# OedonLestrange42/GNURadio-WiFI-ImageTransfer

Hardware: AMD Instinct MI355X
Metric: OFDM demod throughput (complex samples/s), 802.11a RX chain sync->LLR (higher is better)
Workload: dtype f32

## Files before the change

gnuradio-wifi-imagetransfer_amd/csrc/wifirx_api.hip:

```cpp
#include <hip/hip_runtime.h>
#include <emmintrin.h>

#include <algorithm>
#include <array>
#include <atomic>
#include <chrono>
#include <cmath>
#include <cstdio>
#include <cstdlib>
#include <cstring>
#include <condition_variable>
#include <deque>
#include <memory>
#include <mutex>
#include <new>
#include <optional>
#include <thread>
#include <string>
#include <vector>

#include "wifirx.h"
#include "wr_kernels.h"
#include "wr_tx.h"
#include "wr_channel.h"
// ... 38 lines not shown
        p = nullptr;
        bytes = 0;
    }
    int alloc(wifirx_handle* h, size_t n, const char* what)
    {
        reset();
        hipError_t e = Pinned ? hipHostMalloc(&p, n, hipHostMallocDefault) : hipMalloc(&p, n);
        if (e != hipSuccess) { p = nullptr; return oom(h, what, e); }
        bytes = n;
        return WIFIRX_OK;
    }
    int reserve(wifirx_handle* h, size_t need)
    {
        if (bytes >= need) return WIFIRX_OK;
        return Pinned ? alloc(h, need + need / 2, "hipHostMalloc") : alloc(h, need, "hipMalloc");
    }
};
using DevBuf = Buffer<false>;
using PinnedBuf = Buffer<true>;

struct Tunables {
    int32_t  llr_csi = 0;
    int32_t  llr_format = WIFIRX_LLR_F32;
    int32_t  stream_want_idx = 1;
    int32_t  stream_soft = 0;
    int64_t  stream_batch = 0;
    uint32_t decode_small_max = WR_DECODE_SMALL_MAX;
};

struct Environment {
    uint32_t decode_fpw = 0;
    int      decode_ovl = -1;
    int      decode_q = -1;
    int      fail_alloc = 0, alloc_count = 0;
    size_t   decode_budget = 0;
    int      fail_decode_scratch = 0;
    int      fail_carry = 0, carry_count = 0;
};

struct Staging {
    DevBuf iq, frames, idx, llr, car, csi, stats, hbits;
    DevBuf off;
    DevBuf tx_psdu, tx_meta;
    DevBuf ch_meta;
    DevBuf link_meta, link_payload;
    DevBuf link_counts;
    DevBuf iq_clipped;
};

struct DecodeWork {
    DevBuf scratch, max;
    DevBuf perm;
    DevBuf hbits;
};

struct StreamState {
    DevBuf   sbuf;
    DevBuf   native;
    DevBuf   above, A;
    int64_t  sbuf_cap = 0;
    int64_t  sbase = 0;
    int64_t  sfill = 0;
    int64_t  sdetected = 0;
    int64_t  sprocessed = 0;
    int64_t  last_trig = -(1ll << 40);
    std::vector<PendingTrig> pending;
    std::deque<PolledFrame>  queue;
    std::atomic<uint32_t> n_queued{0};
    DevBuf   trig, frames, idx, car, psdu, csi, stats, hbits;
    uint32_t out_cap = 0;
    DevBuf   llr;
    DevBuf   pack;
    PinnedBuf host;
    bool     dead = false;
    std::string dead_msg;
    size_t   push_consumed = 0;
};

struct Job { const void* ptr; size_t n; bool flush; int fmt; float scale; };

struct Worker {
    mutable std::mutex      mu;
    std::condition_variable cv;
    std::thread             thread;
    bool    stop = false, busy = false;
    std::optional<Job> job;
// ... 23 lines not shown
};

namespace {

thread_local std::string g_err;
thread_local bool t_is_worker = false;

int fail(wifirx_handle* h, int code, const std::string& msg)
{
    if (h) { if (t_is_worker) h->w.err_local = msg; else h->err = msg; }
    g_err = msg;
    return code;
}

#define HIP_TRY(h, expr)                                                                       \
    do {                                                                                       \
        hipError_t e_ = (expr);                                                                \
        if (e_ != hipSuccess)                                                                  \
            return fail(h, WIFIRX_EHIP, std::string(#expr) + ": " + hipGetErrorString(e_));   \
    } while (0)

int oom(wifirx_handle* h, const char* what, hipError_t e)
{
    (void)hipGetLastError();
    return fail(h, WIFIRX_ENOMEM, std::string(what) + ": " + hipGetErrorString(e));
}

int read_environment(wifirx_handle* h)
{
    Environment& v = h->env;
    if (const char* e = std::getenv("WIFIRX_DECODE_SMALL_MAX")) h->tune.decode_small_max = (uint32_t)std::strtoul(e, nullptr, 10);
    if (const char* e = std::getenv("WIFIRX_DECODE_FPW")) v.decode_fpw = (uint32_t)std::strtoul(e, nullptr, 10);
    if (const char* e = std::getenv("WIFIRX_DECODE_Q")) v.decode_q = std::atoi(e) != 0;
    if (const char* e = std::getenv("WIFIRX_DECODE_OVL")) { const int m = std::atoi(e); if (m == 0 || m == 2) v.decode_ovl = m; }
    if (const char* e = std::getenv("WIFIRX_TEST_FAIL_ALLOC")) v.fail_alloc = std::atoi(e);
    if (const char* e = std::getenv("WIFIRX_TEST_FAIL_CARRY")) v.fail_carry = std::atoi(e);
    if (const char* e = std::getenv("WIFIRX_TEST_DECODE_BUDGET")) v.decode_budget = (size_t)std::strtoull(e, nullptr, 10);
    if (const char* e = std::getenv("WIFIRX_TEST_FAIL_DECODE_SCRATCH")) v.fail_decode_scratch = std::atoi(e);
    int prio = 0, prio_lo = 0, prio_hi = 0;
    if (const char* e = std::getenv("WIFIRX_STREAM_PRIORITY")) {
        if (hipDeviceGetStreamPriorityRange(&prio_lo, &prio_hi) == hipSuccess) prio = e[0] == 'h' ? prio_hi : e[0] == 'l' ? prio_lo : 0;
        else (void)hipGetLastError();
    }
    return prio;
}

wr::DemodParams params_of(const wifirx_handle* h)
{
    wr::DemodParams p;
    p.bandwidth = h->cfg.bandwidth;
    p.frequency = h->cfg.frequency;
    p.threshold = h->cfg.sensitivity;
    p.min_plateau = h->cfg.min_plateau;
    p.max_sym = h->cfg.max_sym;
    p.llr_bits = h->cfg.llr_bits;
    p.chan_est = h->cfg.chan_est;
    p.llr_csi = h->tune.llr_csi;
    return p;
}

}

static void stream_worker_stop(wifirx_handle* h);
static void stream_worker_wait_idle(wifirx_handle* h);

extern "C" {
// ... 334 lines not shown
```

gnuradio-wifi-imagetransfer_amd/csrc/wifirx_api_decode.inc:

```
static int decode_batch_impl(wifirx_handle* h, uint32_t n_slots, const wifirx_out* out);

extern "C" int wifirx_decode_batch(wifirx_handle* h, uint32_t n_slots, const wifirx_out* out)
{
    if (!h || !out) return WIFIRX_EINVAL;
    stream_worker_wait_idle(h);
    return decode_batch_impl(h, n_slots, out);
}


static int decode_prepass(wifirx_handle* h, uint32_t n_slots, const wifirx_out* out, uint32_t (&pre)[9])
{
    HIP_TRY(h, hipSetDevice(h->device));
    int rc = h->dec.max.reserve(h, 256);
    if (rc) return rc;
    HIP_TRY(h, hipMemsetAsync(h->dec.max.p, 0, 256, h->stream));
    HIP_TRY(h, wr_launch_decode_maxsteps(h->stream, n_slots, h->cfg.max_sym, out->frames, out->psdu_stride,
                                         h->dec.max.as<uint32_t>()));
    HIP_TRY(h, hipMemcpyAsync(pre, h->dec.max.p, sizeof pre, hipMemcpyDeviceToHost, h->stream));
    HIP_TRY(h, hipStreamSynchronize(h->stream));
    return WIFIRX_OK;
}

struct DecodeGroups { uint32_t starts[9]; uint32_t n_virtual; const uint32_t* perm; };

static int decode_group_by_rate(wifirx_handle* h, uint32_t n_slots, const wifirx_out* out, const uint32_t (&pre)[9],
                                uint32_t fpw, DecodeGroups& g)
{
    uint32_t n_rates = 0;
    g.starts[0] = 0;
    for (int e = 0; e < 8; e++) {
        n_rates += pre[1 + e] != 0;
        g.starts[e + 1] = g.starts[e] + (pre[1 + e] + fpw - 1) / fpw * fpw;
    }
    g.n_virtual = n_rates > 1 ? g.starts[8] : n_slots;
    g.perm = nullptr;
    if (n_rates <= 1) return WIFIRX_OK;
    int rc = h->dec.perm.reserve(h, (size_t)g.n_virtual * sizeof(uint32_t));
    if (rc) return rc;
    HIP_TRY(h, hipMemsetAsync(h->dec.perm.p, 0xff, (size_t)g.n_virtual * sizeof(uint32_t), h->stream));
    HIP_TRY(h, wr_launch_decode_perm(h->stream, n_slots, h->cfg.max_sym, out->frames, out->psdu_stride, g.starts,
                                     h->dec.max.as<uint32_t>() + 16, h->dec.perm.as<uint32_t>()));
    g.perm = h->dec.perm.as<const uint32_t>();
    return WIFIRX_OK;
}

static size_t decode_scratch_budget(wifirx_handle* h)
{
    size_t budget = WR_DECODE_SCRATCH_BUDGET;
    size_t mem_free = 0, mem_total = 0;
    if (hipMemGetInfo(&mem_free, &mem_total) == hipSuccess) budget = std::min<size_t>(budget, (mem_free + h->dec.scratch.bytes) / 10 * 7);
    else (void)hipGetLastError();
    if (h->env.decode_budget) budget = std::min<size_t>(budget, h->env.decode_budget);
    return budget;
}

static int decode_alloc_scratch(wifirx_handle* h, size_t stride, size_t want, size_t budget, size_t& n_waves)
{
    n_waves = std::max<size_t>(1, std::min<size_t>(want, budget / stride));
    for (;;) {
        int rc;
        if (h->env.fail_decode_scratch > 0 && h->env.fail_decode_scratch-- > 0) {
            DevBuf none;
            rc = none.reserve(h, SIZE_MAX / 2);
            if (rc == WIFIRX_OK) rc = fail(h, WIFIRX_ENOMEM, "hipMalloc(decode scratch): test hook");
        } else {
            rc = h->dec.scratch.reserve(h, stride * n_waves);
        }
        if (rc == WIFIRX_OK) return WIFIRX_OK;
        if (rc != WIFIRX_ENOMEM || n_waves <= 4) return rc;
        n_waves /= 2;
    }
}

static int decode_batch_impl(wifirx_handle* h, uint32_t n_slots, const wifirx_out* out)
{
    if (!h || !out) return WIFIRX_EINVAL;
    if (!out->on_device) return fail(h, WIFIRX_EINVAL, "wifirx_decode_batch works on device buffers (out->on_device = 1)");
    if (!out->frames || (!out->idx && !out->hbits) || !out->psdu || out->psdu_stride == 0)
        return fail(h, WIFIRX_EINVAL, "frames, hbits or idx, and psdu (with psdu_stride) are required");
    if (reinterpret_cast<uintptr_t>(out->hbits) & 15) return fail(h, WIFIRX_EINVAL, "out->hbits must be 16-byte aligned");
    if (n_slots == 0) return WIFIRX_OK;
    uint32_t pre[9] = { 0 };
    int rc = decode_prepass(h, n_slots, out, pre);
    if (rc || pre[0] == 0) return rc;
    const uint32_t n_steps = pre[0];
    const uint32_t* hbits = out->hbits;
    if (!hbits) {
        rc = h->dec.hbits.reserve(h, (size_t)n_slots * h->cfg.max_sym * 48);
        if (rc) return rc;
        HIP_TRY(h, wr_launch_decode_pack(h->stream, n_slots, h->cfg.max_sym, out->frames, out->idx, out->psdu_stride,
                                         h->dec.hbits.as<uint32_t>(), n_steps));
        hbits = h->dec.hbits.as<const uint32_t>();
    }
    if (n_slots <= h->tune.decode_small_max) {
        const size_t stride = wr::dec_small_slice(n_steps);
        const size_t n_waves = std::min<size_t>(n_slots, WR_DECODE_MAX_WAVES);
        rc = h->dec.scratch.reserve(h, stride * n_waves);
        if (rc) return rc;
        HIP_TRY(h, wr_launch_decode_small(h->stream, n_slots, h->cfg.max_sym, out->frames, hbits, out->psdu,
                                          out->psdu_stride, h->dec.scratch.as<uint8_t>(), stride, n_steps,
                                          (uint32_t)n_waves));
        return WIFIRX_OK;
    }
    uint32_t n_dec = 0;
    for (int e = 0; e < 8; e++) n_dec += pre[1 + e];
    const bool use_q = h->env.decode_q == 1 || (h->env.decode_q < 0 && n_dec >= WR_DECODE_Q_MIN_FRAMES);
    const uint32_t fpw_max = use_q ? WR_DECODE_Q_FRAMES_PER_WAVE : WR_DECODE_FRAMES_PER_WAVE;
    size_t stride = use_q ? wr::dec_q_slice(n_steps, false) : wr::dec_pair_slice(n_steps);
    uint32_t fpw = (uint32_t)std::min<size_t>(fpw_max, std::max<size_t>(1, (n_slots + 1023) / 1024));
    if (use_q && h->env.decode_q < 0) fpw = fpw_max;
    if (h->env.decode_fpw) fpw = std::min<uint32_t>(fpw_max, h->env.decode_fpw);
    DecodeGroups g;
    if ((rc = decode_group_by_rate(h, n_slots, out, pre, fpw, g))) return rc;
    const size_t n_tasks = (g.n_virtual + fpw - 1) / fpw;
    size_t budget = decode_scratch_budget(h);
    const size_t stride_spec = wr::dec_q_slice(n_steps, true);
    const size_t spec_waves = (size_t)h->n_simd * ((pre[7] | pre[8]) ? 2 : WR_DQ_SPEC_WAVES);
    int mode = 0;
    if (use_q) {
        if (h->env.decode_ovl >= 0) mode = h->env.decode_ovl;
        else if (n_tasks >= WR_DECODE_MAX_WAVES / 2 && budget / stride_spec >= spec_waves) mode = 2;
    }
    if (mode == 2) stride = stride_spec;
    size_t n_waves = 0;
    if ((rc = decode_alloc_scratch(h, stride, std::min<size_t>(n_tasks, mode == 2 ? spec_waves : WR_DECODE_MAX_WAVES), budget, n_waves)))
        return rc;
    if (use_q)
        HIP_TRY(h, wr_launch_decode_q(h->stream, n_slots, h->cfg.max_sym, out->frames, hbits, out->psdu,
                                      out->psdu_stride, h->dec.scratch.as<uint8_t>(), stride, n_steps,
                                      (uint32_t)n_waves, fpw, g.perm, g.n_virtual, (pre[7] | pre[8]) != 0, mode));
    else
        HIP_TRY(h, wr_launch_decode(h->stream, n_slots, h->cfg.max_sym, out->frames, hbits, out->psdu,
                                    out->psdu_stride, h->dec.scratch.as<uint8_t>(), stride, n_steps,
                                    (uint32_t)n_waves, fpw, g.perm, g.n_virtual));
    return WIFIRX_OK;
}

static int decode_batch_soft_impl(wifirx_handle* h, uint32_t n_slots, const wifirx_out* out, uint32_t llr_bits, bool bf16);

extern "C" int wifirx_decode_batch_soft(wifirx_handle* h, uint32_t n_slots, const wifirx_out* out)
{
    if (!h || !out) return WIFIRX_EINVAL;
    stream_worker_wait_idle(h);
    if (h->cfg.llr_bits == 0) return fail(h, WIFIRX_EINVAL, "wifirx_decode_batch_soft needs a handle created with llr_bits > 0");
    return decode_batch_soft_impl(h, n_slots, out, h->cfg.llr_bits, h->tune.llr_format == WIFIRX_LLR_BF16);
}

static int decode_batch_soft_impl(wifirx_handle* h, uint32_t n_slots, const wifirx_out* out, uint32_t llr_bits, bool bf16)
{
    if (!out->on_device) return fail(h, WIFIRX_EINVAL, "wifirx_decode_batch_soft works on device buffers (out->on_device = 1)");
    if (!out->frames || !out->llr || !out->psdu || out->psdu_stride == 0)
        return fail(h, WIFIRX_EINVAL, "frames, llr and psdu (with psdu_stride) are required");
    if (reinterpret_cast<uintptr_t>(out->llr) & 15) return fail(h, WIFIRX_EINVAL, "out->llr must be 16-byte aligned");
    if (n_slots == 0) return WIFIRX_OK;
    uint32_t pre[9] = { 0 };
    int rc = decode_prepass(h, n_slots, out, pre);
    if (rc || pre[0] == 0) return rc;
    const uint32_t n_steps = pre[0];
    const uint32_t fpw = 64;
// ... 26 lines not shown
```

gnuradio-wifi-imagetransfer_amd/csrc/wr_decode.h:

```cpp
#pragma once
#include <hip/hip_runtime.h>
#include <stdint.h>

#include "wifirx.h"

namespace wr {

constexpr int RATE_NDBPS[8] = { 24, 36, 48, 72, 96, 144, 192, 216 };
constexpr __host__ __device__ int ndbps_of(int enc) { return RATE_NDBPS[enc]; }
constexpr __host__ __device__ int nbpsc_of(int enc) { return enc < 2 ? 1 : enc < 4 ? 2 : enc < 6 ? 4 : 6; }
constexpr __host__ __device__ int punct_of(int enc) { return enc == 6 ? 1 : (enc & 1) ? 2 : 0; }
constexpr __host__ __device__ int words_per_sym(int enc) { return 2 * nbpsc_of(enc); }

__device__ __forceinline__ int frame_steps(uint32_t flags, int enc, int len, uint32_t psdu_stride, uint32_t max_sym,
                                           uint32_t n_steps_cap)
{
    const int n_dbps = ndbps_of(enc & 7);
    const int n_sym = (16 + 8 * len + 6 + n_dbps - 1) / n_dbps;
    const bool ok = (flags & WIFIRX_F_COMPLETE) && len <= (int)psdu_stride && len <= WIFIRX_MAX_PSDU &&
                    n_sym <= WIFIRX_MAX_SYM && n_sym <= (int)max_sym && (uint32_t)(n_sym * n_dbps) <= n_steps_cap;
    return ok ? n_sym * n_dbps : 0;
}

constexpr int coded_index(int punct, int n_bpsc, int ci)
{
    const int n_cbps = 48 * n_bpsc;
    const int s = (n_bpsc / 2) < 1 ? 1 : (n_bpsc / 2);
    int k = ci;
    if (punct == 1) {
        const int r = ci & 3;
        if (r == 3) return -1;
        k = (ci >> 2) * 3 + r;
    } else if (punct == 2) {
        const int g = ci / 6, r = ci - 6 * g;
        if (r == 3 || r == 4) return -1;
        k = g * 4 + (r < 3 ? r : 3);
    }
    const int i = (n_cbps >> 4) * (k & 15) + (k >> 4);
    return s * (i / s) + (i + n_cbps - (16 * i) / n_cbps) % s;
}

constexpr __host__ __device__ int rotr6(int s, int p) { return ((s >> p) | (s << (6 - p))) & 63; }
constexpr __host__ __device__ int parity_of(int v) { return __builtin_popcount(v) & 1; }

constexpr int RATE_TAB_STRIDE = 216;
struct RateTable { uint32_t e[8 * RATE_TAB_STRIDE]; };
template <typename Entry>
constexpr RateTable make_rate_table(Entry entry)
{
    RateTable t{};
    for (int enc = 0; enc < 8; enc++)
        for (int tt = 0; tt < RATE_TAB_STRIDE; tt++) {
            const int nb = nbpsc_of(enc), pu = punct_of(enc);
            const bool in = tt < ndbps_of(enc);
            const int ja = in ? coded_index(pu, nb, 2 * tt) : -1, jb = in ? coded_index(pu, nb, 2 * tt + 1) : -1;
            t.e[enc * RATE_TAB_STRIDE + tt] = entry(nb, ja) | (entry(nb, jb) << 16);
        }
    return t;
}

struct FinishTables { uint32_t crc[4][256]; uint32_t scr[128]; };

__device__ __forceinline__ void build_finish_tables(FinishTables& ft)
{
    for (int e = threadIdx.x; e < 256; e += blockDim.x) {
        uint32_t c = (uint32_t)e;
#pragma unroll
        for (int k = 0; k < 8; k++) c = (c >> 1) ^ (0xedb88320u & (0u - (c & 1u)));
        ft.crc[0][e] = c;
    }
    __syncthreads();
    for (int e = threadIdx.x; e < 256; e += blockDim.x) {
// ... 61 lines not shown
```

gnuradio-wifi-imagetransfer_amd/csrc/wr_decode.hip:

```cpp
#include <hip/hip_runtime.h>
#include <stdint.h>
#include <type_traits>

#include "wifirx.h"
#include "wr_kernels.h"
#include "wr_decode.h"

namespace wr {

#define WR_DEC_WAVES_PER_SIMD 4
#define WR_DEC_CHUNK      60
#define WR_DEC_NORM_STEPS 120

#define WR_SRC_PUNCT 0x200u
constexpr int bin_of_carrier(int c)
{
    int i = c + 6;
    if (i >= 11) i++;
    if (i >= 25) i++;
    if (i >= 32) i++;
    if (i >= 39) i++;
    if (i >= 53) i++;
    return i;
}
constexpr uint32_t coded_src(int n_bpsc, int j)
{
    if (j < 0) return WR_SRC_PUNCT;
    const int carrier = j / n_bpsc, bit = j - carrier * n_bpsc;
    const int bin = bin_of_carrier(carrier);
    return (uint32_t)(bin & 31) | ((uint32_t)(2 * bit + (bin >> 5)) << 5);
}
__constant__ const RateTable WR_SRC_TABLE = make_rate_table(coded_src);

__device__ __forceinline__ void copy_src_table(uint32_t* tab)
{
    for (int e = threadIdx.x; e < 8 * RATE_TAB_STRIDE; e += blockDim.x) tab[e] = WR_SRC_TABLE.e[e];
}

__device__ __forceinline__ void gather_step(const uint32_t* tile, int sym0, int n_words, const uint32_t* __restrict__ tab_enc,
                                            int n_dbps, uint32_t recip, int t, bool in_range, int& ra, int& rb)
{
    ra = 2; rb = 2;
    if (in_range) {
        const int sym = (int)__umulhi((uint32_t)t, recip);
        const int tt = t - sym * n_dbps;
        const uint32_t e = tab_enc[tt];
        const uint32_t ea = e & 0xffffu, eb = e >> 16;
        const uint32_t* sp = tile + (sym - sym0) * n_words;
        if (!(ea & WR_SRC_PUNCT)) ra = (int)((sp[(ea >> 5) & 15u] >> (ea & 31u)) & 1u);
        if (!(eb & WR_SRC_PUNCT)) rb = (int)((sp[(eb >> 5) & 15u] >> (eb & 31u)) & 1u);
    }
}

#define WR_RECIP32(d) (uint32_t)((0x100000000ull + (d) - 1) / (d))

template <int NB>
__device__ __forceinline__ void pack_symbol(const uint32_t (&by)[12], uint32_t* __restrict__ dst)
{
    uint32_t w[2 * NB];
#pragma unroll
    for (int k = 0; k < 2 * NB; k++) w[k] = 0;
#pragma unroll
    for (int c = 0; c < 48; c++) {
        const int bin = bin_of_carrier(c);
// ... 737 lines not shown
                if (SPEC && blk > 0) {
                    const uint32_t S = rec[(size_t)blk * 64 + lane];
                    bool joined = true;
#pragma unroll
                    for (int h = 0; h < 4; h++) joined = joined && st[h] == (int)((S >> (8 * h)) & 63u) && fb[h] >= blk;
                    if (__all(joined)) break;
                }
            }
#undef WR_DQ_PICK
        }
        __threadfence_block();
#pragma unroll
        for (int h = 0; h < 4; h++) {
            if (n_data[h] > 0) {
                const uint32_t slot = slot_of[h];
                finish_frame<256>(dbits + 64 * h + lane, frames[slot].psdu_len, psdu_all + (size_t)slot * psdu_stride,
                                  ((reinterpret_cast<uintptr_t>(psdu_all) | psdu_stride) & 3) == 0, frames + slot, frames[slot].flags, ft);
            }
        }
    }
}

__device__ __forceinline__ uint32_t crc32_update(uint32_t c, uint32_t byte)
{
    c ^= byte;
#pragma unroll
    for (int k = 0; k < 8; k++) c = (c >> 1) ^ (0xedb88320u & (0u - (c & 1u)));
    return c;
}

__global__ __launch_bounds__(256)
void decode_small_kernel(uint32_t n_slots, uint32_t max_sym, wifirx_frame* __restrict__ frames,
                         const uint32_t* __restrict__ hbits_all, uint8_t* __restrict__ psdu_all, uint32_t psdu_stride,
                         uint8_t* __restrict__ scratch, size_t scratch_stride, uint32_t n_steps_cap, uint32_t n_waves_total)
{
    __shared__ uint32_t tile_all[4][60 * 12];
    __shared__ uint32_t src_tab[8 * RATE_TAB_STRIDE];
    copy_src_table(src_tab);
    __syncthreads();
    const int lane = threadIdx.x & 63;
    const int wv = threadIdx.x >> 6;
    const uint32_t wave = blockIdx.x * 4 + wv;
    if (wave >= n_waves_total) return;
    uint32_t* tile = tile_all[wv];
    uint8_t* const slice = scratch + (size_t)wave * scratch_stride;
    uint64_t* dec = reinterpret_cast<uint64_t*>(slice);
    uint64_t* words = reinterpret_cast<uint64_t*>(slice + dec_small_words_at(n_steps_cap));

    const int s = lane, u = s & 1, p0 = s >> 1, p1 = (s >> 1) | 32;
    const int f0 = (p0 << 1) | u;
    const int a0 = __builtin_popcount(f0 & 0155) & 1, b0 = __builtin_popcount(f0 & 0117) & 1;
    const uint32_t recip_tab[8] = { WR_RECIP32(24), WR_RECIP32(36), WR_RECIP32(48), WR_RECIP32(72),
                                    WR_RECIP32(96), WR_RECIP32(144), WR_RECIP32(192), WR_RECIP32(216) };

    for (uint32_t slot = wave; slot < n_slots; slot += n_waves_total) {
        const wifirx_frame fr = frames[slot];
        const int enc = fr.encoding & 7, psdu_len = fr.psdu_len;
        const int n_data = frame_steps(fr.flags, enc, psdu_len, psdu_stride, max_sym, n_steps_cap);
        if (n_data == 0) continue;
        const int n_dbps = ndbps_of(enc);
        const int n_sym = __builtin_amdgcn_readfirstlane(n_data / n_dbps);
        const int n_words = words_per_sym(enc);
        const uint32_t* fhb = hbits_all + (size_t)slot * max_sym * 12;
        const uint32_t recip = recip_tab[enc];
        const uint32_t* tab_enc = src_tab + enc * RATE_TAB_STRIDE;

        int pm = (s == 0) ? 0 : (1 << 24);
        for (int sym0 = 0; sym0 < n_sym; sym0 += 60) {
            const int nsy = n_sym - sym0 < 60 ? n_sym - sym0 : 60;
            const int nw = nsy * n_words;
            __builtin_amdgcn_wave_barrier();
            for (int o = lane; o < nw; o += 64) tile[o] = fhb[sym0 * n_words + o];
            __builtin_amdgcn_wave_barrier();
            const int t_hi = (sym0 + nsy) * n_dbps;
            for (int t0 = sym0 * n_dbps; t0 < t_hi; t0 += WR_DEC_CHUNK) {
                const int t = t0 + lane;
                int ra, rb;
                gather_step(tile, sym0, n_words, tab_enc, n_dbps, recip, t, lane < WR_DEC_CHUNK && t < t_hi, ra, rb);
                const uint64_t A1 = __ballot(ra == 1), AV = __ballot(ra != 2);
                const uint64_t B1 = __ballot(rb == 1), BV = __ballot(rb != 2);
                const int jn = t_hi - t0 < WR_DEC_CHUNK ? t_hi - t0 : WR_DEC_CHUNK;
                uint64_t mydec = 0;
                for (int j = 0; j < jn; j++) {
                    const int sa = (int)((A1 >> j) & 1), va = (int)((AV >> j) & 1);
                    const int sb = (int)((B1 >> j) & 1), vb = (int)((BV >> j) & 1);
                    const int bm0 = (va & (sa ^ a0)) + (vb & (sb ^ b0));
                    const int bm1 = (va + vb) - bm0;
                    const int m0 = __shfl(pm, p0, 64) + bm0;
                    const int m1 = __shfl(pm, p1, 64) + bm1;
                    const bool sel = m1 < m0;
                    pm = sel ? m1 : m0;
                    const uint64_t d = __ballot(sel);
// ... 71 lines not shown
                            uint32_t psdu_stride, uint32_t* __restrict__ out)
{
    uint32_t best = 0;
    uint32_t cnt[8] = { 0, 0, 0, 0, 0, 0, 0, 0 };
    const uint32_t n_round = (n_slots + 63u) & ~63u;
    for (uint32_t i = blockIdx.x * blockDim.x + threadIdx.x; i < n_round; i += gridDim.x * blockDim.x) {
        int enc = -1;
        if (i < n_slots) {
            const wifirx_frame fr = frames[i];
            const uint32_t v = (uint32_t)frame_steps(fr.flags, fr.encoding & 7, fr.psdu_len, psdu_stride, max_sym, 0xffffffffu);
            if (v) {
                best = v > best ? v : best;
                enc = fr.encoding & 7;
            }
        }
#pragma unroll
        for (int e = 0; e < 8; e++) cnt[e] += (uint32_t)__builtin_popcountll(__ballot(enc == e));
    }
#pragma unroll
    for (int k = 1; k < 64; k <<= 1) {
        uint32_t o = __shfl_xor(best, k, 64);
        best = o > best ? o : best;
    }
    if ((threadIdx.x & 63) == 0) {
        if (best) atomicMax(out, best);
#pragma unroll
        for (int e = 0; e < 8; e++) if (cnt[e]) atomicAdd(out + 1 + e, cnt[e]);
    }
}

struct PermStarts { uint32_t s[8]; };
__global__ __launch_bounds__(256)
void decode_perm_kernel(uint32_t n_slots, uint32_t max_sym, const wifirx_frame* __restrict__ frames, uint32_t psdu_stride,
                        PermStarts start, uint32_t* __restrict__ cursor, uint32_t* __restrict__ perm)
{
    const int lane = threadIdx.x & 63;
    const uint32_t n_round = (n_slots + 63u) & ~63u;
    for (uint32_t i = blockIdx.x * blockDim.x + threadIdx.x; i < n_round; i += gridDim.x * blockDim.x) {
        int enc = -1;
        if (i < n_slots) {
            const wifirx_frame fr = frames[i];
            if (frame_steps(fr.flags, fr.encoding & 7, fr.psdu_len, psdu_stride, max_sym, 0xffffffffu)) enc = fr.encoding & 7;
        }
#pragma unroll
        for (int e = 0; e < 8; e++) {
            const uint64_t m = __ballot(enc == e);
            if (m == 0) continue;
            uint32_t at = 0;
            if (lane == (int)__builtin_ctzll(m)) at = atomicAdd(cursor + e, (uint32_t)__builtin_popcountll(m));
            at = (uint32_t)__builtin_amdgcn_readlane((int)at, (int)__builtin_ctzll(m));
            if (enc == e) perm[start.s[e] + at + (uint32_t)__builtin_popcountll(m & ((1ull << lane) - 1ull))] = i;
        }
    }
}

}

extern "C" hipError_t wr_launch_decode_maxsteps(hipStream_t st, uint32_t n_slots, uint32_t max_sym,
                                                const wifirx_frame* frames, uint32_t psdu_stride, uint32_t* out)
{
    if (n_slots == 0) return hipSuccess;
    uint32_t blocks = (n_slots + 255) / 256;
    if (blocks > 1024) blocks = 1024;
    hipLaunchKernelGGL(wr::decode_maxsteps_kernel, dim3(blocks), dim3(256), 0, st, n_slots, max_sym, frames, psdu_stride, out);
    return hipGetLastError();
}

extern "C" hipError_t wr_launch_decode_pack(hipStream_t st, uint32_t n_slots, uint32_t max_sym, const wifirx_frame* frames,
                                            const uint8_t* idx, uint32_t psdu_stride, uint32_t* hbits, uint32_t n_steps_cap)
{
    if (n_slots == 0) return hipSuccess;
    uint32_t blocks = (n_slots + 3) / 4;
    if (blocks > 16384) blocks = 16384;
    hipLaunchKernelGGL(wr::decode_pack_kernel, dim3(blocks), dim3(256), 0, st, n_slots, max_sym, frames, idx, psdu_stride,
                       hbits, n_steps_cap);
    return hipGetLastError();
}

extern "C" hipError_t wr_launch_decode(hipStream_t st, uint32_t n_slots, uint32_t max_sym, wifirx_frame* frames,
                                       const uint32_t* hbits, uint8_t* psdu, uint32_t psdu_stride, uint8_t* scratch,
                                       size_t scratch_stride, uint32_t n_steps_cap, uint32_t n_waves, uint32_t frames_per_wave,
                                       const uint32_t* perm, uint32_t n_virtual)
{
    if (n_slots == 0 || n_waves == 0) return hipSuccess;
    if (!perm) n_virtual = n_slots;
    hipLaunchKernelGGL(wr::decode_kernel, dim3((n_waves + 3) / 4), dim3(256), 0, st, n_slots, max_sym, frames, hbits, psdu,
                       psdu_stride, scratch, scratch_stride, n_steps_cap, n_waves, frames_per_wave, perm, n_virtual);
    return hipGetLastError();
}

extern "C" hipError_t wr_launch_decode_q(hipStream_t st, uint32_t n_slots, uint32_t max_sym, wifirx_frame* frames,
                                         const uint32_t* hbits, uint8_t* psdu, uint32_t psdu_stride, uint8_t* scratch,
                                         size_t scratch_stride, uint32_t n_steps_cap, uint32_t n_waves, uint32_t frames_per_wave,
                                         const uint32_t* perm, uint32_t n_virtual, int has_64qam, int mode)
{
    if (n_slots == 0 || n_waves == 0) return hipSuccess;
    if (!perm) n_virtual = n_slots;
#define WR_LAUNCH_Q(ROWS, MODE) hipLaunchKernelGGL((wr::decode_q_kernel<ROWS, MODE>), dim3((n_waves + 3) / 4), dim3(256), 0, st, n_slots, max_sym, \
                                                   frames, hbits, psdu, psdu_stride, scratch, scratch_stride, n_steps_cap, n_waves, frames_per_wave, perm, n_virtual)
    if (has_64qam) { if (mode == 2) WR_LAUNCH_Q(48, 2); else WR_LAUNCH_Q(48, 0); }
    else           { if (mode == 2) WR_LAUNCH_Q(32, 2); else WR_LAUNCH_Q(32, 0); }
#undef WR_LAUNCH_Q
    return hipGetLastError();
}

extern "C" hipError_t wr_launch_decode_perm(hipStream_t st, uint32_t n_slots, uint32_t max_sym, const wifirx_frame* frames,
                                            uint32_t psdu_stride, const uint32_t* starts8, uint32_t* cursor8, uint32_t* perm)
{
    if (n_slots == 0) return hipSuccess;
    wr::PermStarts ps;
    for (int e = 0; e < 8; e++) ps.s[e] = starts8[e];
    uint32_t blocks = (n_slots + 255) / 256;
    if (blocks > 2048) blocks = 2048;
    hipLaunchKernelGGL(wr::decode_perm_kernel, dim3(blocks), dim3(256), 0, st, n_slots, max_sym, frames, psdu_stride, ps, cursor8, perm);
    return hipGetLastError();
}

extern "C" hipError_t wr_launch_decode_small(hipStream_t st, uint32_t n_slots, uint32_t max_sym, wifirx_frame* frames,
                                             const uint32_t* hbits, uint8_t* psdu, uint32_t psdu_stride, uint8_t* scratch,
                                             size_t scratch_stride, uint32_t n_steps_cap, uint32_t n_waves)
{
    if (n_slots == 0 || n_waves == 0) return hipSuccess;
    hipLaunchKernelGGL(wr::decode_small_kernel, dim3((n_waves + 3) / 4), dim3(256), 0, st, n_slots, max_sym, frames, hbits, psdu,
                       psdu_stride, scratch, scratch_stride, n_steps_cap, n_waves);
    return hipGetLastError();
}
```

gnuradio-wifi-imagetransfer_amd/csrc/wr_kernels.h:

```cpp
#pragma once
#include <hip/hip_runtime.h>
#include <stdint.h>

#include "wifirx.h"

#ifndef WR_WAVES_PER_BLOCK
#define WR_WAVES_PER_BLOCK 1
#endif
#ifndef WR_DEMOD_WAVES_PER_SIMD
#define WR_DEMOD_WAVES_PER_SIMD 4
#endif
#ifndef WR_DEMOD_WAVES_PER_SIMD_STA
#define WR_DEMOD_WAVES_PER_SIMD_STA 4
#endif
#define WR_STREAM_SPAN     16
#define WR_DECODE_MAX_WAVES 4096
#define WR_DQ_SPEC_WAVES 3
#define WR_DECODE_SMALL_MAX 16384
#define WR_DECODE_FRAMES_PER_WAVE 128
#define WR_DECODE_Q_FRAMES_PER_WAVE 256
#define WR_DECODE_Q_MIN_FRAMES 600000
#define WR_DECODE_SCRATCH_BUDGET (24ull << 30)

namespace wr {

struct DemodParams {
    double   bandwidth;
    double   frequency;
    float    threshold;
    int32_t  min_plateau;
    uint32_t max_sym;
    uint32_t llr_bits;
    int32_t  chan_est;
    int32_t  llr_csi;
};

struct DemodOut {
    wifirx_frame* frames;
    uint8_t*      idx;
    float*        llr;
    float2*       carrier;
    float2*       csi;
    float4*       sym_stats;
    uint32_t*     hbits;
};

constexpr __host__ __device__ size_t dec_small_words_at(size_t n) { return n * 8; }
constexpr __host__ __device__ size_t dec_small_slice(size_t n) { return dec_small_words_at(n) + (n / 60 + 4) * 8; }
constexpr __host__ __device__ size_t dec_pair_dbits_at(size_t n) { return n * 64 * 16; }
constexpr __host__ __device__ size_t dec_pair_slice(size_t n) { return dec_pair_dbits_at(n) + (n / 32 + 2) * 128 * 4; }
constexpr __host__ __device__ size_t dec_q_dbits_at(size_t n) { return n * 64 * 32; }
constexpr __host__ __device__ size_t dec_q_rec_at(size_t n) { return dec_q_dbits_at(n) + (n / 32 + 2) * 256 * 4; }
constexpr __host__ __device__ size_t dec_q_slice(size_t n, bool spec) { return dec_q_rec_at(n) + (spec ? (n / 96 + 2) * 64 * 4 : 0); }
constexpr __host__ __device__ size_t dec_soft_dbits_at(size_t n) { return n * 64 * 8; }
constexpr __host__ __device__ size_t dec_soft_slice(size_t n) { return dec_soft_dbits_at(n) + (n / 32 + 2) * 64 * 4; }

struct StreamTrig {
    int64_t pos;
    int64_t usable;
    float   cfo;
    int32_t pad;
};

}

static inline bool wr_demod_wants_x(const wr::DemodParams* prm, const wr::DemodOut* out)
{
    return out->carrier != nullptr || out->sym_stats != nullptr || out->idx == nullptr || out->llr == nullptr || prm->llr_csi != 0;
}

extern "C" {
hipError_t wr_launch_demod_batch_x(hipStream_t st, const float2* iq, uint32_t slot_len, uint32_t n_slots,
                                   const wr::DemodParams* prm, const wr::DemodOut* out, const uint64_t* slot_off);
hipError_t wr_launch_demod_stream_x(hipStream_t st, const float2* x, int64_t n_samp, const wr::StreamTrig* trig,
                                    uint32_t n_trig, const wr::DemodParams* prm, const float2* A, const wr::DemodOut* out);
hipError_t wr_launch_demod_batch(hipStream_t st, const float2* iq, uint32_t slot_len, uint32_t n_slots,
                                 const wr::DemodParams* prm, const wr::DemodOut* out, const uint64_t* slot_off);
hipError_t wr_launch_demod_batch_bf16(hipStream_t st, const float2* iq, uint32_t slot_len, uint32_t n_slots,
                                      const wr::DemodParams* prm, const wr::DemodOut* out, const uint64_t* slot_off);
hipError_t wr_launch_demod_batch_bf16_x(hipStream_t st, const float2* iq, uint32_t slot_len, uint32_t n_slots,
                                        const wr::DemodParams* prm, const wr::DemodOut* out, const uint64_t* slot_off);
hipError_t wr_launch_synth(hipStream_t st, const float2* templates, uint32_t n_templates, uint32_t frame_len,
                           float2* slots, uint32_t slot_len, uint32_t n_slots, uint32_t lead, float gain,
                           float noise, float cfo_max, uint64_t seed, float* cfo_out);
hipError_t wr_launch_decode_maxsteps(hipStream_t st, uint32_t n_slots, uint32_t max_sym,
                                     const wifirx_frame* frames, uint32_t psdu_stride, uint32_t* out);
hipError_t wr_launch_decode_pack(hipStream_t st, uint32_t n_slots, uint32_t max_sym, const wifirx_frame* frames,
                                 const uint8_t* idx, uint32_t psdu_stride, uint32_t* hbits, uint32_t n_steps_cap);
hipError_t wr_launch_decode(hipStream_t st, uint32_t n_slots, uint32_t max_sym, wifirx_frame* frames,
                            const uint32_t* hbits, uint8_t* psdu, uint32_t psdu_stride, uint8_t* scratch,
                            size_t scratch_stride, uint32_t n_steps_cap, uint32_t n_waves, uint32_t frames_per_wave,
                            const uint32_t* perm, uint32_t n_virtual);
hipError_t wr_launch_decode_q(hipStream_t st, uint32_t n_slots, uint32_t max_sym, wifirx_frame* frames,
                              const uint32_t* hbits, uint8_t* psdu, uint32_t psdu_stride, uint8_t* scratch,
                              size_t scratch_stride, uint32_t n_steps_cap, uint32_t n_waves, uint32_t frames_per_wave,
                              const uint32_t* perm, uint32_t n_virtual, int has_64qam, int mode);
hipError_t wr_launch_decode_perm(hipStream_t st, uint32_t n_slots, uint32_t max_sym, const wifirx_frame* frames,
                                 uint32_t psdu_stride, const uint32_t* starts8, uint32_t* cursor8, uint32_t* perm);
hipError_t wr_launch_decode_soft(hipStream_t st, int nb, uint32_t n_slots, uint32_t max_sym, uint32_t llr_bits,
                                 wifirx_frame* frames, const float* llr, uint8_t* psdu, uint32_t psdu_stride,
                                 uint8_t* scratch, size_t scratch_stride, uint32_t n_steps_cap, uint32_t n_waves,
                                 const uint32_t* perm, uint32_t n_virtual, uint32_t task_lo, uint32_t task_hi);
hipError_t wr_launch_decode_soft_bf16(hipStream_t st, int nb, uint32_t n_slots, uint32_t max_sym, uint32_t llr_bits,
                                      wifirx_frame* frames, const uint16_t* llr, uint8_t* psdu, uint32_t psdu_stride,
                                      uint8_t* scratch, size_t scratch_stride, uint32_t n_steps_cap, uint32_t n_waves,
                                      const uint32_t* perm, uint32_t n_virtual, uint32_t task_lo, uint32_t task_hi);
hipError_t wr_launch_decode_small(hipStream_t st, uint32_t n_slots, uint32_t max_sym, wifirx_frame* frames,
                                  const uint32_t* hbits, uint8_t* psdu, uint32_t psdu_stride, uint8_t* scratch,
                                  size_t scratch_stride, uint32_t n_steps_cap, uint32_t n_waves);
hipError_t wr_launch_stream_detect(hipStream_t st, const float2* x, int64_t n_samp, int64_t tile0,
                                   int64_t n_tiles, float thr, uint64_t* masks, float2* A);
hipError_t wr_launch_demod_stream(hipStream_t st, const float2* x, int64_t n_samp, const wr::StreamTrig* trig,
                                  uint32_t n_trig, const wr::DemodParams* prm, const float2* A, const wr::DemodOut* out);
}
```

Baseline: 433.4 billion.

## Add syndrome-based fast path that skips Viterbi for error-free frames

Adds a fast pre-pass kernel that checks the convolutional-code syndrome of each frame's hard bits (BPSK/QPSK/16QAM rate-1/2). When the syndrome is zero, it inverts the code directly and finishes the frame. Frames that settle this way are marked, and the Viterbi decode and permutation kernels then skip them, so only dirty frames go through full decoding. This is a decode-side change; the stated metric is the demod chain (sync->LLR), so it may not affect that measurement. It also adds an extra pass and scratch allocation on every decode call.

```diff
diff --git a/gnuradio-wifi-imagetransfer_amd/csrc/wifirx_api.hip b/gnuradio-wifi-imagetransfer_amd/csrc/wifirx_api.hip
--- a/gnuradio-wifi-imagetransfer_amd/csrc/wifirx_api.hip
+++ b/gnuradio-wifi-imagetransfer_amd/csrc/wifirx_api.hip
@@ -94,6 +94,8 @@
     uint32_t decode_fpw = 0;
     int      decode_ovl = -1;
     int      decode_q = -1;
+    bool     decode_fast = true;
+    bool     decode_no_viterbi = false;
     int      fail_alloc = 0, alloc_count = 0;
     size_t   decode_budget = 0;
     int      fail_decode_scratch = 0;
@@ -114,6 +116,7 @@
     DevBuf scratch, max;
     DevBuf perm;
     DevBuf hbits;
+    DevBuf settled, fast;
 };
 
 struct StreamState {
@@ -203,6 +206,8 @@
     if (const char* e = std::getenv("WIFIRX_DECODE_SMALL_MAX")) h->tune.decode_small_max = (uint32_t)std::strtoul(e, nullptr, 10);
     if (const char* e = std::getenv("WIFIRX_DECODE_FPW")) v.decode_fpw = (uint32_t)std::strtoul(e, nullptr, 10);
     if (const char* e = std::getenv("WIFIRX_DECODE_Q")) v.decode_q = std::atoi(e) != 0;
+    if (const char* e = std::getenv("WIFIRX_DECODE_FAST")) v.decode_fast = std::atoi(e) != 0;
+    if (const char* e = std::getenv("WIFIRX_TEST_DECODE_NO_VITERBI")) v.decode_no_viterbi = std::atoi(e) != 0;
     if (const char* e = std::getenv("WIFIRX_DECODE_OVL")) { const int m = std::atoi(e); if (m == 0 || m == 2) v.decode_ovl = m; }
     if (const char* e = std::getenv("WIFIRX_TEST_FAIL_ALLOC")) v.fail_alloc = std::atoi(e);
     if (const char* e = std::getenv("WIFIRX_TEST_FAIL_CARRY")) v.fail_carry = std::atoi(e);
diff --git a/gnuradio-wifi-imagetransfer_amd/csrc/wifirx_api_decode.inc b/gnuradio-wifi-imagetransfer_amd/csrc/wifirx_api_decode.inc
--- a/gnuradio-wifi-imagetransfer_amd/csrc/wifirx_api_decode.inc
+++ b/gnuradio-wifi-imagetransfer_amd/csrc/wifirx_api_decode.inc
@@ -21,25 +21,53 @@
     return WIFIRX_OK;
 }
 
+static int decode_fast_pass(wifirx_handle* h, uint32_t n_slots, const wifirx_out* out, const uint32_t*& hbits,
+                            uint32_t (&pre)[9], uint32_t (&dirty)[9])
+{
+    HIP_TRY(h, hipSetDevice(h->device));
+    int rc = h->dec.max.reserve(h, 256);
+    if (rc) return rc;
+    HIP_TRY(h, hipMemsetAsync(h->dec.max.p, 0, 256, h->stream));
+    if (!hbits) {
+        if ((rc = h->dec.hbits.reserve(h, (size_t)n_slots * h->cfg.max_sym * 48))) return rc;
+        HIP_TRY(h, wr_launch_decode_pack(h->stream, n_slots, h->cfg.max_sym, out->frames, out->idx, out->psdu_stride,
+                                         h->dec.hbits.as<uint32_t>(), 0xffffffffu));
+        hbits = h->dec.hbits.as<const uint32_t>();
+    }
+    const size_t stride = wr::dec_fast_slice(h->cfg.max_sym);
+    const size_t n_waves = std::max<size_t>(1, std::min<size_t>({ (n_slots + 63) / 64, (size_t)h->n_simd * 8, WR_FAST_SCRATCH_BUDGET / stride }));
+    if ((rc = h->dec.settled.reserve(h, n_slots))) return rc;
+    if ((rc = h->dec.fast.reserve(h, stride * n_waves))) return rc;
+    HIP_TRY(h, wr_launch_decode_fast(h->stream, n_slots, h->cfg.max_sym, out->frames, hbits, out->psdu, out->psdu_stride,
+                                     h->dec.fast.as<uint8_t>(), stride, (uint32_t)n_waves, h->dec.settled.as<uint8_t>(),
+                                     h->dec.max.as<uint32_t>()));
+    uint32_t cnt[WR_FAST_DIRTY_AT + 9];
+    HIP_TRY(h, hipMemcpyAsync(cnt, h->dec.max.p, sizeof cnt, hipMemcpyDeviceToHost, h->stream));
+    HIP_TRY(h, hipStreamSynchronize(h->stream));
+    for (int k = 0; k < 9; k++) { pre[k] = cnt[k]; dirty[k] = cnt[WR_FAST_DIRTY_AT + k]; }
+    return WIFIRX_OK;
+}
+
 struct DecodeGroups { uint32_t starts[9]; uint32_t n_virtual; const uint32_t* perm; };
 
-static int decode_group_by_rate(wifirx_handle* h, uint32_t n_slots, const wifirx_out* out, const uint32_t (&pre)[9],
-                                uint32_t fpw, DecodeGroups& g)
+static int decode_group_by_rate(wifirx_handle* h, uint32_t n_slots, const wifirx_out* out, const uint32_t (&cnt)[9],
+                                uint32_t fpw, DecodeGroups& g, const uint8_t* settled = nullptr, bool build = true)
 {
     uint32_t n_rates = 0;
     g.starts[0] = 0;
     for (int e = 0; e < 8; e++) {
-        n_rates += pre[1 + e] != 0;
-        g.starts[e + 1] = g.starts[e] + (pre[1 + e] + fpw - 1) / fpw * fpw;
-    }
-    g.n_virtual = n_rates > 1 ? g.starts[8] : n_slots;
+        n_rates += cnt[1 + e] != 0;
+        g.starts[e + 1] = g.starts[e] + (cnt[1 + e] + fpw - 1) / fpw * fpw;
+    }
+    const bool permuted = n_rates > 1 || settled;
+    g.n_virtual = permuted ? g.starts[8] : n_slots;
     g.perm = nullptr;
-    if (n_rates <= 1) return WIFIRX_OK;
+    if (!permuted || !build) return WIFIRX_OK;
     int rc = h->dec.perm.reserve(h, (size_t)g.n_virtual * sizeof(uint32_t));
     if (rc) return rc;
     HIP_TRY(h, hipMemsetAsync(h->dec.perm.p, 0xff, (size_t)g.n_virtual * sizeof(uint32_t), h->stream));
     HIP_TRY(h, wr_launch_decode_perm(h->stream, n_slots, h->cfg.max_sym, out->frames, out->psdu_stride, g.starts,
-                                     h->dec.max.as<uint32_t>() + 16, h->dec.perm.as<uint32_t>()));
+                                     h->dec.max.as<uint32_t>() + 16, h->dec.perm.as<uint32_t>(), settled));
     g.perm = h->dec.perm.as<const uint32_t>();
     return WIFIRX_OK;
 }
@@ -80,11 +108,17 @@
         return fail(h, WIFIRX_EINVAL, "frames, hbits or idx, and psdu (with psdu_stride) are required");
     if (reinterpret_cast<uintptr_t>(out->hbits) & 15) return fail(h, WIFIRX_EINVAL, "out->hbits must be 16-byte aligned");
     if (n_slots == 0) return WIFIRX_OK;
-    uint32_t pre[9] = { 0 };
-    int rc = decode_prepass(h, n_slots, out, pre);
+    uint32_t pre[9] = { 0 }, dirty[9] = { 0 };
+    const uint32_t* hbits = out->hbits;
+    const bool fast = h->env.decode_fast;
+    int rc = fast ? decode_fast_pass(h, n_slots, out, hbits, pre, dirty) : decode_prepass(h, n_slots, out, pre);
     if (rc || pre[0] == 0) return rc;
+    if (fast && h->env.decode_no_viterbi) return WIFIRX_OK;
+    if (!fast) std::copy(pre, pre + 9, dirty);
     const uint32_t n_steps = pre[0];
-    const uint32_t* hbits = out->hbits;
+    uint32_t n_dec = 0, n_dirty = 0;
+    for (int e = 0; e < 8; e++) { n_dec += pre[1 + e]; n_dirty += dirty[1 + e]; }
+    const uint8_t* settled = n_dirty != n_dec ? h->dec.settled.as<const uint8_t>() : nullptr;
     if (!hbits) {
         rc = h->dec.hbits.reserve(h, (size_t)n_slots * h->cfg.max_sym * 48);
         if (rc) return rc;
@@ -97,13 +131,12 @@
         const size_t n_waves = std::min<size_t>(n_slots, WR_DECODE_MAX_WAVES);
         rc = h->dec.scratch.reserve(h, stride * n_waves);
         if (rc) return rc;
+        if (n_dirty == 0) return WIFIRX_OK;
         HIP_TRY(h, wr_launch_decode_small(h->stream, n_slots, h->cfg.max_sym, out->frames, hbits, out->psdu,
                                           out->psdu_stride, h->dec.scratch.as<uint8_t>(), stride, n_steps,
-                                          (uint32_t)n_waves));
+                                          (uint32_t)n_waves, settled));
         return WIFIRX_OK;
     }
-    uint32_t n_dec = 0;
-    for (int e = 0; e < 8; e++) n_dec += pre[1 + e];
     const bool use_q = h->env.decode_q == 1 || (h->env.decode_q < 0 && n_dec >= WR_DECODE_Q_MIN_FRAMES);
     const uint32_t fpw_max = use_q ? WR_DECODE_Q_FRAMES_PER_WAVE : WR_DECODE_FRAMES_PER_WAVE;
     size_t stride = use_q ? wr::dec_q_slice(n_steps, false) : wr::dec_pair_slice(n_steps);
@@ -111,7 +144,7 @@
     if (use_q && h->env.decode_q < 0) fpw = fpw_max;
     if (h->env.decode_fpw) fpw = std::min<uint32_t>(fpw_max, h->env.decode_fpw);
     DecodeGroups g;
-    if ((rc = decode_group_by_rate(h, n_slots, out, pre, fpw, g))) return rc;
+    decode_group_by_rate(h, n_slots, out, pre, fpw, g, nullptr, false);
     const size_t n_tasks = (g.n_virtual + fpw - 1) / fpw;
     size_t budget = decode_scratch_budget(h);
     const size_t stride_spec = wr::dec_q_slice(n_steps, true);
@@ -125,6 +158,9 @@
     size_t n_waves = 0;
     if ((rc = decode_alloc_scratch(h, stride, std::min<size_t>(n_tasks, mode == 2 ? spec_waves : WR_DECODE_MAX_WAVES), budget, n_waves)))
         return rc;
+    if (n_dirty == 0) return WIFIRX_OK;
+    if ((rc = decode_group_by_rate(h, n_slots, out, dirty, fpw, g, settled))) return rc;
+    n_waves = std::min<size_t>(n_waves, (g.n_virtual + fpw - 1) / fpw);
     if (use_q)
         HIP_TRY(h, wr_launch_decode_q(h->stream, n_slots, h->cfg.max_sym, out->frames, hbits, out->psdu,
                                       out->psdu_stride, h->dec.scratch.as<uint8_t>(), stride, n_steps,
diff --git a/gnuradio-wifi-imagetransfer_amd/csrc/wr_decode.h b/gnuradio-wifi-imagetransfer_amd/csrc/wr_decode.h
--- a/gnuradio-wifi-imagetransfer_amd/csrc/wr_decode.h
+++ b/gnuradio-wifi-imagetransfer_amd/csrc/wr_decode.h
@@ -38,6 +38,25 @@
     }
     const int i = (n_cbps >> 4) * (k & 15) + (k >> 4);
     return s * (i / s) + (i + n_cbps - (16 * i) / n_cbps) % s;
+}
+
+#define WR_SRC_PUNCT 0x200u
+constexpr int bin_of_carrier(int c)
+{
+    int i = c + 6;
+    if (i >= 11) i++;
+    if (i >= 25) i++;
+    if (i >= 32) i++;
+    if (i >= 39) i++;
+    if (i >= 53) i++;
+    return i;
+}
+constexpr uint32_t coded_src(int n_bpsc, int j)
+{
+    if (j < 0) return WR_SRC_PUNCT;
+    const int carrier = j / n_bpsc, bit = j - carrier * n_bpsc;
+    const int bin = bin_of_carrier(carrier);
+    return (uint32_t)(bin & 31) | ((uint32_t)(2 * bit + (bin >> 5)) << 5);
 }
 
 constexpr __host__ __device__ int rotr6(int s, int p) { return ((s >> p) | (s << (6 - p))) & 63; }
diff --git a/gnuradio-wifi-imagetransfer_amd/csrc/wr_decode.hip b/gnuradio-wifi-imagetransfer_amd/csrc/wr_decode.hip
--- a/gnuradio-wifi-imagetransfer_amd/csrc/wr_decode.hip
+++ b/gnuradio-wifi-imagetransfer_amd/csrc/wr_decode.hip
@@ -12,24 +12,6 @@
 #define WR_DEC_CHUNK      60
 #define WR_DEC_NORM_STEPS 120
 
-#define WR_SRC_PUNCT 0x200u
-constexpr int bin_of_carrier(int c)
-{
-    int i = c + 6;
-    if (i >= 11) i++;
-    if (i >= 25) i++;
-    if (i >= 32) i++;
-    if (i >= 39) i++;
-    if (i >= 53) i++;
-    return i;
-}
-constexpr uint32_t coded_src(int n_bpsc, int j)
-{
-    if (j < 0) return WR_SRC_PUNCT;
-    const int carrier = j / n_bpsc, bit = j - carrier * n_bpsc;
-    const int bin = bin_of_carrier(carrier);
-    return (uint32_t)(bin & 31) | ((uint32_t)(2 * bit + (bin >> 5)) << 5);
-}
 __constant__ const RateTable WR_SRC_TABLE = make_rate_table(coded_src);
 
 __device__ __forceinline__ void copy_src_table(uint32_t* tab)
@@ -833,7 +815,8 @@
 __global__ __launch_bounds__(256)
 void decode_small_kernel(uint32_t n_slots, uint32_t max_sym, wifirx_frame* __restrict__ frames,
                          const uint32_t* __restrict__ hbits_all, uint8_t* __restrict__ psdu_all, uint32_t psdu_stride,
-                         uint8_t* __restrict__ scratch, size_t scratch_stride, uint32_t n_steps_cap, uint32_t n_waves_total)
+                         uint8_t* __restrict__ scratch, size_t scratch_stride, uint32_t n_steps_cap, uint32_t n_waves_total,
+                         const uint8_t* __restrict__ settled)
 {
     __shared__ uint32_t tile_all[4][60 * 12];
     __shared__ uint32_t src_tab[8 * RATE_TAB_STRIDE];
@@ -858,7 +841,7 @@
         const wifirx_frame fr = frames[slot];
         const int enc = fr.encoding & 7, psdu_len = fr.psdu_len;
         const int n_data = frame_steps(fr.flags, enc, psdu_len, psdu_stride, max_sym, n_steps_cap);
-        if (n_data == 0) continue;
+        if (n_data == 0 || (settled && settled[slot])) continue;
         const int n_dbps = ndbps_of(enc);
         const int n_sym = __builtin_amdgcn_readfirstlane(n_data / n_dbps);
         const int n_words = words_per_sym(enc);
@@ -996,13 +979,14 @@
 struct PermStarts { uint32_t s[8]; };
 __global__ __launch_bounds__(256)
 void decode_perm_kernel(uint32_t n_slots, uint32_t max_sym, const wifirx_frame* __restrict__ frames, uint32_t psdu_stride,
-                        PermStarts start, uint32_t* __restrict__ cursor, uint32_t* __restrict__ perm)
+                        PermStarts start, uint32_t* __restrict__ cursor, uint32_t* __restrict__ perm,
+                        const uint8_t* __restrict__ settled)
 {
     const int lane = threadIdx.x & 63;
     const uint32_t n_round = (n_slots + 63u) & ~63u;
     for (uint32_t i = blockIdx.x * blockDim.x + threadIdx.x; i < n_round; i += gridDim.x * blockDim.x) {
         int enc = -1;
-        if (i < n_slots) {
+        if (i < n_slots && !(settled && settled[i])) {
             const wifirx_frame fr = frames[i];
             if (frame_steps(fr.flags, fr.encoding & 7, fr.psdu_len, psdu_stride, max_sym, 0xffffffffu)) enc = fr.encoding & 7;
         }
@@ -1069,23 +1053,24 @@
 }
 
 extern "C" hipError_t wr_launch_decode_perm(hipStream_t st, uint32_t n_slots, uint32_t max_sym, const wifirx_frame* frames,
-                                            uint32_t psdu_stride, const uint32_t* starts8, uint32_t* cursor8, uint32_t* perm)
+                                            uint32_t psdu_stride, const uint32_t* starts8, uint32_t* cursor8, uint32_t* perm,
+                                            const uint8_t* settled)
 {
     if (n_slots == 0) return hipSuccess;
     wr::PermStarts ps;
     for (int e = 0; e < 8; e++) ps.s[e] = starts8[e];
     uint32_t blocks = (n_slots + 255) / 256;
     if (blocks > 2048) blocks = 2048;
-    hipLaunchKernelGGL(wr::decode_perm_kernel, dim3(blocks), dim3(256), 0, st, n_slots, max_sym, frames, psdu_stride, ps, cursor8, perm);
+    hipLaunchKernelGGL(wr::decode_perm_kernel, dim3(blocks), dim3(256), 0, st, n_slots, max_sym, frames, psdu_stride, ps, cursor8, perm, settled);
     return hipGetLastError();
 }
 
 extern "C" hipError_t wr_launch_decode_small(hipStream_t st, uint32_t n_slots, uint32_t max_sym, wifirx_frame* frames,
                                              const uint32_t* hbits, uint8_t* psdu, uint32_t psdu_stride, uint8_t* scratch,
-                                             size_t scratch_stride, uint32_t n_steps_cap, uint32_t n_waves)
+                                             size_t scratch_stride, uint32_t n_steps_cap, uint32_t n_waves, const uint8_t* settled)
 {
     if (n_slots == 0 || n_waves == 0) return hipSuccess;
     hipLaunchKernelGGL(wr::decode_small_kernel, dim3((n_waves + 3) / 4), dim3(256), 0, st, n_slots, max_sym, frames, hbits, psdu,
-                       psdu_stride, scratch, scratch_stride, n_steps_cap, n_waves);
+                       psdu_stride, scratch, scratch_stride, n_steps_cap, n_waves, settled);
     return hipGetLastError();
 }
diff --git a/gnuradio-wifi-imagetransfer_amd/csrc/wr_decode_fast.hip b/gnuradio-wifi-imagetransfer_amd/csrc/wr_decode_fast.hip
--- /dev/null
+++ b/gnuradio-wifi-imagetransfer_amd/csrc/wr_decode_fast.hip
@@ -0,0 +1,142 @@
+#include <hip/hip_runtime.h>
+#include <stdint.h>
+
+#include "wifirx.h"
+#include "wr_kernels.h"
+#include "wr_decode.h"
+
+namespace wr {
+
+template <int NB>
+__device__ __forceinline__ bool settle_frame(const uint32_t* __restrict__ fhb, int n_sym, uint32_t* db)
+{
+    constexpr int NW = 2 * NB;
+    constexpr int ND = 24 * NB;
+    constexpr int CH = NB == 1 ? 24 : 48;
+    constexpr int SB = 16 / NW;
+    constexpr uint64_t MASK = (1ull << CH) - 1ull;
+    uint64_t ha = 0, hb = 0;
+    uint64_t acc = 0;
+    int fill = 0, wi = 0;
+    for (int s0 = 0; s0 < n_sym; s0 += SB) {
+        uint32_t w[16];
+#pragma unroll
+        for (int k = 0; k < 16; k += 4) {
+            uint4 v = make_uint4(0u, 0u, 0u, 0u);
+            if (s0 + k / NW < n_sym) v = *reinterpret_cast<const uint4*>(fhb + s0 * NW + k);
+            w[k] = v.x; w[k + 1] = v.y; w[k + 2] = v.z; w[k + 3] = v.w;
+        }
+#pragma unroll
+        for (int q = 0; q < SB; q++) {
+            if (s0 + q >= n_sym) break;
+#pragma unroll
+            for (int c = 0; c < ND / CH; c++) {
+                uint64_t a = 0, b = 0;
+#pragma unroll
+                for (int i = 0; i < CH; i++) {
+                    const uint32_t ea = coded_src(NB, coded_index(0, NB, 2 * (c * CH + i)));
+                    const uint32_t eb = coded_src(NB, coded_index(0, NB, 2 * (c * CH + i) + 1));
+                    a |= (uint64_t)((w[q * NW + (ea >> 5)] >> (ea & 31u)) & 1u) << i;
+                    b |= (uint64_t)((w[q * NW + (eb >> 5)] >> (eb & 31u)) & 1u) << i;
+                }
+                const uint64_t xa = (a << 6) | ha, xb = (b << 6) | hb;
+                const uint64_t syn = ((xa >> 6) ^ (xa >> 5) ^ (xa >> 4) ^ (xa >> 3) ^ xa ^
+                                      (xb >> 6) ^ (xb >> 4) ^ (xb >> 3) ^ (xb >> 1) ^ xb) & MASK;
+                if (syn) return false;
+                const uint64_t u = ((xa >> 4) ^ (xa >> 2) ^ (xb >> 6) ^ (xb >> 5) ^ (xb >> 4) ^ (xb >> 3) ^ (xb >> 2)) & MASK;
+                ha = (xa >> CH) & 63u;
+                hb = (xb >> CH) & 63u;
+#pragma unroll
+                for (int p = 0; p < CH; p += 32) {
+                    const int nb = CH - p < 32 ? CH - p : 32;
+                    acc |= (uint64_t)(uint32_t)(u >> p) << fill;
+                    fill += nb;
+                    if (fill >= 32) {
+                        db[(size_t)wi * 64] = (uint32_t)acc;
+                        wi++;
+                        acc >>= 32;
+                        fill -= 32;
+                    }
+                }
+            }
+        }
+    }
+    if (fill) db[(size_t)wi * 64] = (uint32_t)acc;
+    return true;
+}
+
+__global__ __launch_bounds__(256)
+void decode_fast_kernel(uint32_t n_slots, uint32_t max_sym, wifirx_frame* __restrict__ frames,
+                        const uint32_t* __restrict__ hbits_all, uint8_t* __restrict__ psdu_all, uint32_t psdu_stride,
+                        uint8_t* __restrict__ scratch, size_t scratch_stride, uint32_t n_waves_total,
+                        uint8_t* __restrict__ settled, uint32_t* __restrict__ counts)
+{
+    __shared__ FinishTables ft;
+    build_finish_tables(ft);
+    const int lane = threadIdx.x & 63;
+    const uint32_t wave = blockIdx.x * 4 + (threadIdx.x >> 6);
+    if (wave >= n_waves_total) return;
+    uint32_t* const db = reinterpret_cast<uint32_t*>(scratch + (size_t)wave * scratch_stride) + lane;
+    const uint32_t hb_stride = max_sym * 12;
+    const bool dword_ok = ((reinterpret_cast<uintptr_t>(psdu_all) | psdu_stride) & 3) == 0;
+    uint32_t best = 0, best_dirty = 0;
+    uint32_t cnt[8] = { 0, 0, 0, 0, 0, 0, 0, 0 }, cnt_dirty[8] = { 0, 0, 0, 0, 0, 0, 0, 0 };
+    const uint32_t n_round = (n_slots + 63u) & ~63u;
+    for (uint32_t i = wave * 64 + lane; i < n_round; i += n_waves_total * 64) {
+        int enc = -1;
+        bool done = false;
+        if (i < n_slots) {
+            const wifirx_frame fr = frames[i];
+            const int e = fr.encoding & 7;
+            const uint32_t steps = (uint32_t)frame_steps(fr.flags, e, fr.psdu_len, psdu_stride, max_sym, 0xffffffffu);
+            if (steps) {
+                enc = e;
+                best = steps > best ? steps : best;
+                const uint32_t* fhb = hbits_all + (size_t)i * hb_stride;
+                const int n_sym = (int)steps / ndbps_of(e);
+                if (e == 0)      done = settle_frame<1>(fhb, n_sym, db);
+                else if (e == 2) done = settle_frame<2>(fhb, n_sym, db);
+                else if (e == 4) done = settle_frame<4>(fhb, n_sym, db);
+                if (done) {
+                    __threadfence_block();
+                    finish_frame<64>(db, fr.psdu_len, psdu_all + (size_t)i * psdu_stride, dword_ok, frames + i, fr.flags, ft);
+                } else {
+                    best_dirty = steps > best_dirty ? steps : best_dirty;
+                }
+            }
+            settled[i] = done ? 1 : 0;
+        }
+#pragma unroll
+        for (int e = 0; e < 8; e++) {
+            cnt[e] += (uint32_t)__builtin_popcountll(__ballot(enc == e));
+            cnt_dirty[e] += (uint32_t)__builtin_popcountll(__ballot(enc == e && !done));
+        }
+    }
+#pragma unroll
+    for (int k = 1; k < 64; k <<= 1) {
+        const uint32_t o = __shfl_xor(best, k, 64), od = __shfl_xor(best_dirty, k, 64);
+        best = o > best ? o : best;
+        best_dirty = od > best_dirty ? od : best_dirty;
+    }
+    if (lane == 0) {
+        if (best) atomicMax(counts, best);
+        if (best_dirty) atomicMax(counts + WR_FAST_DIRTY_AT, best_dirty);
+#pragma unroll
+        for (int e = 0; e < 8; e++) {
+            if (cnt[e]) atomicAdd(counts + 1 + e, cnt[e]);
+            if (cnt_dirty[e]) atomicAdd(counts + WR_FAST_DIRTY_AT + 1 + e, cnt_dirty[e]);
+        }
+    }
+}
+
+}
+
+extern "C" hipError_t wr_launch_decode_fast(hipStream_t st, uint32_t n_slots, uint32_t max_sym, wifirx_frame* frames,
+                                            const uint32_t* hbits, uint8_t* psdu, uint32_t psdu_stride, uint8_t* scratch,
+                                            size_t scratch_stride, uint32_t n_waves, uint8_t* settled, uint32_t* counts)
+{
+    if (n_slots == 0 || n_waves == 0) return hipSuccess;
+    hipLaunchKernelGGL(wr::decode_fast_kernel, dim3((n_waves + 3) / 4), dim3(256), 0, st, n_slots, max_sym, frames, hbits, psdu,
+                       psdu_stride, scratch, scratch_stride, n_waves, settled, counts);
+    return hipGetLastError();
+}
diff --git a/gnuradio-wifi-imagetransfer_amd/csrc/wr_kernels.h b/gnuradio-wifi-imagetransfer_amd/csrc/wr_kernels.h
--- a/gnuradio-wifi-imagetransfer_amd/csrc/wr_kernels.h
+++ b/gnuradio-wifi-imagetransfer_amd/csrc/wr_kernels.h
@@ -21,6 +21,8 @@
 #define WR_DECODE_Q_FRAMES_PER_WAVE 256
 #define WR_DECODE_Q_MIN_FRAMES 600000
 #define WR_DECODE_SCRATCH_BUDGET (24ull << 30)
+#define WR_FAST_DIRTY_AT 32
+#define WR_FAST_SCRATCH_BUDGET (256ull << 20)
 
 namespace wr {
 
@@ -52,6 +54,7 @@
 constexpr __host__ __device__ size_t dec_q_dbits_at(size_t n) { return n * 64 * 32; }
 constexpr __host__ __device__ size_t dec_q_rec_at(size_t n) { return dec_q_dbits_at(n) + (n / 32 + 2) * 256 * 4; }
 constexpr __host__ __device__ size_t dec_q_slice(size_t n, bool spec) { return dec_q_rec_at(n) + (spec ? (n / 96 + 2) * 64 * 4 : 0); }
+constexpr __host__ __device__ size_t dec_fast_slice(size_t max_sym) { return (3 * max_sym + 2) * 64 * 4; }
 constexpr __host__ __device__ size_t dec_soft_dbits_at(size_t n) { return n * 64 * 8; }
 constexpr __host__ __device__ size_t dec_soft_slice(size_t n) { return dec_soft_dbits_at(n) + (n / 32 + 2) * 64 * 4; }
 
@@ -96,7 +99,11 @@
                               size_t scratch_stride, uint32_t n_steps_cap, uint32_t n_waves, uint32_t frames_per_wave,
                               const uint32_t* perm, uint32_t n_virtual, int has_64qam, int mode);
 hipError_t wr_launch_decode_perm(hipStream_t st, uint32_t n_slots, uint32_t max_sym, const wifirx_frame* frames,
-                                 uint32_t psdu_stride, const uint32_t* starts8, uint32_t* cursor8, uint32_t* perm);
+                                 uint32_t psdu_stride, const uint32_t* starts8, uint32_t* cursor8, uint32_t* perm,
+                                 const uint8_t* settled);
+hipError_t wr_launch_decode_fast(hipStream_t st, uint32_t n_slots, uint32_t max_sym, wifirx_frame* frames,
+                                 const uint32_t* hbits, uint8_t* psdu, uint32_t psdu_stride, uint8_t* scratch,
+                                 size_t scratch_stride, uint32_t n_waves, uint8_t* settled, uint32_t* counts);
 hipError_t wr_launch_decode_soft(hipStream_t st, int nb, uint32_t n_slots, uint32_t max_sym, uint32_t llr_bits,
                                  wifirx_frame* frames, const float* llr, uint8_t* psdu, uint32_t psdu_stride,
                                  uint8_t* scratch, size_t scratch_stride, uint32_t n_steps_cap, uint32_t n_waves,
@@ -107,7 +114,7 @@
                                       const uint32_t* perm, uint32_t n_virtual, uint32_t task_lo, uint32_t task_hi);
 hipError_t wr_launch_decode_small(hipStream_t st, uint32_t n_slots, uint32_t max_sym, wifirx_frame* frames,
                                   const uint32_t* hbits, uint8_t* psdu, uint32_t psdu_stride, uint8_t* scratch,
-                                  size_t scratch_stride, uint32_t n_steps_cap, uint32_t n_waves);
+                                  size_t scratch_stride, uint32_t n_steps_cap, uint32_t n_waves, const uint8_t* settled);
 hipError_t wr_launch_stream_detect(hipStream_t st, const float2* x, int64_t n_samp, int64_t tile0,
                                    int64_t n_tiles, float thr, uint64_t* masks, float2* A);
 hipError_t wr_launch_demod_stream(hipStream_t st, const float2* x, int64_t n_samp, const wr::StreamTrig* trig,
```

After: 432.6 billion. About the same (-0.2%).
